# RedhawkSDR/psk_soft

Measured on AMD Instinct MI355X. Metric: complex IQ Msamples/s, QPSK 8 sps, 4096 ch; % HBM roofline at 1/2/4/8 GPUs, higher is better.
Workload: dtype f32

## Files before the change

### psk_soft_amd/csrc/psk_capi.cpp

```cpp
#include <hip/hip_runtime_api.h>
#include <hip/hip_vector_types.h>

#include <atomic>
#include <cmath>
#include <condition_variable>
#include <cstdio>
#include <cstdlib>
#include <cstring>
#include <functional>
#include <mutex>
#include <new>
#include <string>
#include <thread>
#include <vector>

#include "psk_acquire.h"
#include "psk_ctl.h"
#include "psk_gather.h"
#include "psk_plan.h"
#include "psk_quality.h"
#include "psk_soft_hip.h"
#include "psk_tune.h"

namespace psk {
// ... 369 lines not shown
    hipStream_t up_stream = nullptr;
    hipEvent_t ev_up[kPlanSlots] = {};
    int opt_up_stream = 1;
    bool ev_used[kPlanSlots] = {};
    int slot = 0;
    bool opt_qpsk_sign_map = false;
    hipStream_t stream = nullptr;
    hipStream_t aux[kAuxStreams] = {};
    hipEvent_t aux_fork = nullptr, aux_join[kAuxStreams] = {};
    int opt_fork = 1;
    int opt_deferred = 0;
    bool deferred_pending = false;
    uint64_t deferred_sig = 0;
    uint32_t deferred_ch0 = 0, deferred_nch = 0;
    hipStream_t deferred_stream = nullptr;
    hipEvent_t slot_aux_ev[kPlanSlots][kAuxStreams] = {};
    bool slot_aux_used[kPlanSlots][kAuxStreams] = {};
    hipStream_t slot_stream[kPlanSlots] = {};
    uint32_t slot_ch0[kPlanSlots] = {}, slot_nch[kPlanSlots] = {};
    int opt_tiled = 1;
    psk::TileInfo *d_tiles = nullptr;
    float *d_traw = nullptr, *d_test = nullptr;
    float2 *d_ts = nullptr;
    size_t tile_cap = 0, tile_sym_cap = 0;
    size_t pf_cap = 0, pf_sym_cap = 0;
    psk::PfScratch pf{};
    int opt_pfit = 1;
    int pf_second_ttl = 0;
    int opt_ties_in_place = 1;
    int opt_trace = 0;
    int opt_validate = 0;
    int opt_split = 2;
    int opt_pipe = 1;
    hipStream_t pipe_st[2] = {};
    hipEvent_t pipe_ev[kPipeEvents] = {};
    void *d_pipe_carry = nullptr;
    float *d_pipe_y = nullptr;
    size_t pipe_cap = 0;
    void *d_wide_rec = nullptr, *d_wide_stat = nullptr;
    size_t wide_rec_cap = 0, wide_stat_cap = 0;
    double *d_wide_symE = nullptr;
    size_t wide_symE_cap = 0;
    hipEvent_t tile_ev = nullptr;
    hipStream_t tile_stream = nullptr;
    bool tile_ev_used = false;
    int opt_far_fit = 0;
    float *d_far_y = nullptr;
    uint32_t far_rows_cap = 0, far_rows_used = 0;
    std::vector<uint32_t> far_row;
    bool poisoned = false;
    StreamScratch cvt[kCvtScratch];
    uint64_t cvt_calls = 0;
    StreamScratch gat[kGatherScratch];
    GatherDescSlot gdesc[kGatherDescSlots];
    uint64_t gat_calls = 0;
    int gdesc_turn = 0;
    float *d_tune_tab = nullptr;
    int opt_diag_gather_only = 0;
    int opt_quality = 0;
    psk_soft_quality_t *d_quality = nullptr;
    std::vector<psk_soft_quality_t> quality_dry;
    PassRing<psk::QualityDesc, psk::QualityPartial, kQualitySlots> qpass;
    struct QualitySnap {
        uint16_t M, S;
        uint8_t diff;
    };
// ... 988 lines not shown
    float *const carry_y = h->d_pipe_y + (size_t)kPipeMaxYLen * s.off;
    const uint32_t y_pipe = ring_floats(s.max_n, 512u);
    int e = 0;
    PSK_HIP(hipEventRecord(h->pipe_ev[e], st));
    PSK_HIP(hipStreamWaitEvent(h->pipe_st[0], h->pipe_ev[e], 0));
    PSK_HIP(hipStreamWaitEvent(h->pipe_st[1], h->pipe_ev[e], 0));
    e++;
    for (uint32_t t0 = 0; t0 < T; t0 += tr) {
        const uint32_t nt = T - t0 < tr ? T - t0 : tr;
        PSK_HIP(mark(r, st, "pipe_front", S, H, s.off, cnt, nt, y_len, r_len));
        PSK_HIP(psk::launch_tile_front(S, class_H(H), r.d_plans, l, r.ch0, cnt, nt, h->d_state, h->d_ring, h->lim.ring_cap, r_len, h->d_tiles,
                                       h->d_traw, h->d_ts, h->pf.chan, t0, st));
        PSK_HIP(hipEventRecord(h->pipe_ev[e], st));
        PSK_HIP(hipStreamWaitEvent(h->pipe_st[0], h->pipe_ev[e], 0));
        e++;
        PSK_HIP(mark(r, h->pipe_st[0], "pipe_fit", S, H, s.off, cnt, nt, y_pipe, 0));
        PSK_HIP(psk::launch_tile_fit_range(r.d_plans, l, r.ch0, cnt, h->d_state, h->d_ring, h->lim.ring_cap, h->d_yv, h->lim.fit_cap, y_pipe,
                                           h->d_tiles, h->d_traw, h->d_ts, h->d_test, carry, carry_y, t0, nt, h->pipe_st[0]));
        PSK_HIP(hipEventRecord(h->pipe_ev[e], h->pipe_st[0]));
        PSK_HIP(hipStreamWaitEvent(h->pipe_st[1], h->pipe_ev[e], 0));
        e++;
        PSK_HIP(mark(r, h->pipe_st[1], "pipe_back", S, H, s.off, cnt, nt, y_pipe, 0));
        PSK_HIP(psk::launch_tile_back(r.d_plans, l, r.ch0, cnt, nt, h->d_state, h->d_tiles, h->d_ts, h->d_test, t0, 1u, h->pipe_st[1]));
    }
    PSK_HIP(hipEventRecord(h->pipe_ev[e], h->pipe_st[1]));
    PSK_HIP(hipStreamWaitEvent(st, h->pipe_ev[e], 0));
    return PSK_SOFT_OK;
}
psk_soft_status enqueue_class(const Round &r, int S, int H, hipStream_t st)
{
    psk_soft_handle *const h = r.h;
    const LaunchSet &s = r.res.cls[S][H];
    const uint32_t *const l = r.d_list + s.off;
    const uint32_t y_len = ring_floats(s.max_n, psk::ering_dynamic(S) ? 256u : 512u);
    const uint32_t r_len = class_H(H) == 1 ? ((s.max_A + 128u + 1u) & ~1u) : 0u;
    if (s.tiled && s.piped)
        PSK_TRY(enqueue_piped(r, s, S, H, y_len, r_len, st));
    else if (s.tiled)
        PSK_TRY(enqueue_tiled(r, s, {"tile_front", "pfit", "tile_fit", "tile_back", S, H, y_len, r_len, r_len}, Front::window_class, Fit::lds, st));
    const psk::PktFormat *const f = class_pkt(H);
    for (int exact = s.tiled ? 1 : 0; exact <= 1; exact++) {
        if (exact && diag_no_tail())
            break;
        PSK_HIP(mark(r, st, exact ? "fast (exact tier)" : "fast (screened tier)", S, H, s.off, s.cnt, 0, y_len, r_len));
        if (f)
            PSK_HIP(psk::launch_fast_pkt((int)f->id, S, exact, r.d_plans, l, r.ch0, s.cnt, h->d_state, h->d_ring, h->lim.ring_cap, h->d_yv,
                                         h->lim.fit_cap, y_len, r_len, st));
        else
            PSK_HIP(psk::launch_fast(S, class_H(H), exact, r.d_plans, l, r.ch0, s.cnt, h->d_state, h->d_ring, h->lim.ring_cap, h->d_yv,
                                     h->lim.fit_cap, y_len, r_len, st));
    }
    if (r.deferred && f)
        PSK_HIP(psk::launch_seq_pkt((int)f->id, r.d_plans, l, r.ch0, s.cnt, h->d_state, h->d_ring, h->lim.ring_cap, h->d_yv, h->lim.fit_cap, st));
    else if (r.deferred)
        PSK_HIP(psk::launch_seq(r.d_plans, l, r.ch0, s.cnt, h->d_state, h->d_ring, h->lim.ring_cap, h->d_yv, h->lim.fit_cap, st));
    return PSK_SOFT_OK;
}
psk_soft_status enqueue_join_and_tail(Round &r, int used_aux)
{
    psk_soft_handle *const h = r.h;
    const hipStream_t st = r.stream;
    if (r.deferred) {
        for (int a = 0; a < used_aux && a < kAuxStreams; a++) {
            if (!h->slot_aux_ev[r.slot][a])
                PSK_HIP(hipEventCreateWithFlags(&h->slot_aux_ev[r.slot][a], hipEventDisableTiming));
            PSK_HIP(hipEventRecord(h->slot_aux_ev[r.slot][a], h->aux[a]));
            h->slot_aux_used[r.slot][a] = true;
// ... 183 lines not shown
    h->nch = n_channels;
    h->user = lim;
    h->lim.ring_cap = lim.max_window_samples;
    h->lim.fit_cap = lim.max_phase_avg + 1;
    h->lim.fast_fit_max = kFastFitMax;
    h->lim.force_seq = false;
    h->lim.far_fit = false;
    h->ctl.resize(n_channels);
    h->ctl_next.resize(n_channels);
    h->last_mode.assign(n_channels, psk::PLAN_SKIP);
    h->device = device;
    h->dry = (device == PSK_SOFT_DEVICE_NONE);
    if (h->dry) {
        h->quality_dry.assign(n_channels, psk_soft_quality_t{});
        h->acquire_dry.assign(n_channels, psk_soft_acquire_t{});
    }
    if (const char *e = std::getenv("PSK_SOFT_TIME_TILED"))
        h->opt_tiled = std::atoi(e) < 0 ? 0 : std::atoi(e) > 2 ? 2 : std::atoi(e);
    if (const char *e = std::getenv("PSK_SOFT_FAR_FIT"))
        h->opt_far_fit = std::atoi(e) != 0;
    h->lim.far_fit = h->opt_far_fit != 0;
    if (const char *e = std::getenv("PSK_SOFT_TIES_IN_PLACE"))
        h->opt_ties_in_place = std::atoi(e) != 0;
    if (const char *e = std::getenv("PSK_SOFT_TRACE_LAUNCHES"))
        h->opt_trace = std::atoi(e);
    if (const char *e = std::getenv("PSK_SOFT_VALIDATE"))
        h->opt_validate = std::atoi(e);
    if (const char *e = std::getenv("PSK_SOFT_DIAG_GATHER_ONLY"))
        h->opt_diag_gather_only = std::atoi(e) != 0;
    if (const char *e = std::getenv("PSK_SOFT_SPLIT_CLASSES"))
        h->opt_split = std::atoi(e) < 0 ? 0 : std::atoi(e) > 16 ? 16 : std::atoi(e);
    if (const char *e = std::getenv("PSK_SOFT_PIPELINED"))
        h->opt_pipe = std::atoi(e) < 0 ? 0 : std::atoi(e) > 2 ? 2 : std::atoi(e);
    if (const char *e = std::getenv("PSK_SOFT_DEFERRED_JOIN"))
        h->opt_deferred = std::atoi(e) != 0;
    if (const char *e = std::getenv("PSK_SOFT_STAMP"))
        h->opt_stamp = std::atoi(e) != 0;
    if (const char *e = std::getenv("PSK_SOFT_PARALLEL_FIT"))
        h->opt_pfit = std::atoi(e) < 0 ? 0 : std::atoi(e) > 2 ? 2 : std::atoi(e);
    if (!h->dry) {
        int ndev = 0;
        hipError_t e = hipGetDeviceCount(&ndev);
        if (e != hipSuccess || ndev <= 0 || device < 0 || device >= ndev) {
            delete h;
            return fail(PSK_SOFT_ERR_NO_DEVICE,
                        std::string("psk_soft_create: no usable HIP device (") +
                            (e != hipSuccess ? hipGetErrorString(e) : "device index out of range") + ")");
        }
        hipDeviceProp_t prop;
        if (hipSetDevice(device) != hipSuccess || hipGetDeviceProperties(&prop, device) != hipSuccess) {
            delete h;
            return fail(PSK_SOFT_ERR_NO_DEVICE, "psk_soft_create: hipSetDevice failed");
        }
        if (std::strncmp(prop.gcnArchName, "gfx950", 6) != 0) {
            delete h;
            return fail(PSK_SOFT_ERR_NO_DEVICE,
                        std::string("psk_soft_create: kernels are built for gfx950 only, device is ") + prop.gcnArchName);
        }
        auto bail = [&](const char *what, hipError_t e2) {
            std::string msg = std::string("psk_soft_create: ") + what + ": " + hipGetErrorString(e2);
            psk_soft_destroy(h);
            return fail(PSK_SOFT_ERR_HIP, msg);
        };
        hipError_t e2;
        if ((e2 = hipStreamCreateWithFlags(&h->stream, hipStreamNonBlocking)) != hipSuccess)
            return bail("hipStreamCreate", e2);
        size_t state_b = sizeof(psk::ChanState) * (size_t)n_channels;
        size_t ring_b = sizeof(float2) * 2u * (size_t)h->lim.ring_cap * n_channels;
        size_t yv_b = sizeof(float) * (size_t)h->lim.fit_cap * n_channels;
        if ((e2 = hipMalloc((void **)&h->d_state, state_b)) != hipSuccess) return bail("hipMalloc state", e2);
        if ((e2 = hipMalloc((void **)&h->d_ring, ring_b)) != hipSuccess) return bail("hipMalloc ring", e2);
        if ((e2 = hipMalloc((void **)&h->d_yv, yv_b)) != hipSuccess) return bail("hipMalloc yvals", e2);
        std::vector<psk::ChanState> init(n_channels);
        std::memset(init.data(), 0, state_b);
        for (auto &s : init) s.lf_den = 1.0f;
        if ((e2 = hipMemcpy(h->d_state, init.data(), state_b, hipMemcpyHostToDevice)) != hipSuccess)
            return bail("hipMemcpy state", e2);
        if ((e2 = hipMemset(h->d_ring, 0, ring_b)) != hipSuccess) return bail("hipMemset", e2);
        if ((e2 = hipMemset(h->d_yv, 0, yv_b)) != hipSuccess) return bail("hipMemset", e2);
        if ((e2 = hipMalloc((void **)&h->d_quality, sizeof(psk_soft_quality_t) * (size_t)n_channels)) != hipSuccess)
            return bail("hipMalloc quality", e2);
        if ((e2 = hipMemset(h->d_quality, 0, sizeof(psk_soft_quality_t) * (size_t)n_channels)) != hipSuccess) return bail("hipMemset", e2);
        if ((e2 = hipMalloc((void **)&h->d_acquire, sizeof(psk_soft_acquire_t) * (size_t)n_channels)) != hipSuccess)
            return bail("hipMalloc acquire", e2);
        if ((e2 = hipMemset(h->d_acquire, 0, sizeof(psk_soft_acquire_t) * (size_t)n_channels)) != hipSuccess) return bail("hipMemset", e2);
        for (int s = 0; s < kPlanSlots; s++) {
            char *hb = nullptr, *db = nullptr;
            if ((e2 = hipHostMalloc((void **)&hb, slot_bytes(n_channels))) != hipSuccess)
                return bail("hipHostMalloc plans", e2);
            std::memset(hb, 0, psk::kPlanHeaderBytes);
            h->h_plans[s] = reinterpret_cast<psk::ChanPlan *>(hb + psk::kPlanHeaderBytes);
// ... 1450 lines not shown
```

### psk_soft_amd/csrc/psk_fast_kernel.h

```cpp
#ifndef PSK_FAST_KERNEL_H
#define PSK_FAST_KERNEL_H

#include <mutex>

#include "psk_fast_loop.h"

namespace psk {

PSK_HD int hist_blocks_for(uint32_t A) { return A <= 128u ? 1 : A <= 256u ? 2 : A <= 512u ? 4 : 8; }

template <bool FAR = false>
PSK_DEV void call_prologue(const ChanPlan &p, const ChanState *st, const float *yv, uint32_t fit_cap, float *yring, uint32_t ymask,
                           int lane, FastCarry &cy)
{
    const uint32_t len0 = p.lf_len0;
    for (uint32_t j = lane; j < len0; j += kWave) yring[j & ymask] = yv[(p.lf_head + j) % fit_cap];
    if constexpr (FAR)
        far_ring_fence();
    else
        wave_lds_fence();
    cy.ySum = st->lf_ySum;
    cy.xySum = st->lf_xySum;
    cy.est = st->phaseEstimate;
    cy.last_re = st->last_re;
// ... 85 lines not shown
            st->stat_chain = cy.stat_chain;
            st->stat_pfit = 0u;
        }
    }
}

#ifndef PSK_WAVES_PER_SIMD
#define PSK_WAVES_PER_SIMD 4
#endif
#ifndef PSK_WAVES_PER_SIMD_H0
#define PSK_WAVES_PER_SIMD_H0 2
#endif
#ifndef PSK_WAVES_PER_SIMD_H2
#define PSK_WAVES_PER_SIMD_H2 1
#endif
template <int SV, int HV, bool EXACT>
__global__ __launch_bounds__(64, ((HV == 0 && SV <= 5 && !EXACT) ? 4 : (HV == 0 && SV <= 10 && !EXACT) ? PSK_WAVES_PER_SIMD_H0 : (HV == 1 && SV <= 10 && !EXACT) ? PSK_WAVES_PER_SIMD : (HV == 2 && SV <= 10 && !EXACT) ? PSK_WAVES_PER_SIMD_H2 : (HV == 4 && SV <= 8 && !EXACT && PSK_DBUF) ? 2 : 1)) void psk_fast_kernel(const ChanPlan *__restrict__ plans, const uint32_t *__restrict__ list, uint32_t ch0,
                                                      ChanState *__restrict__ states, float2 *__restrict__ rings,
                                                      uint32_t ring_cap, float *__restrict__ yvs, uint32_t fit_cap,
                                                      uint32_t y_len, uint32_t r_len)
{
    extern __shared__ __attribute__((aligned(16))) float lds_dyn[];
    constexpr bool kDyn = ering_dynamic(SV);
    float *const yring = lds_dyn;
    const uint32_t ymask = y_len - 1u;
    ERingT<kDyn> er;
    if constexpr (kDyn) {
        er.mem = lds_dyn + y_len;
        er.set_len((int)r_len);
    } else {
        __shared__ __attribute__((aligned(16))) float ering_s[(SV != 0 && HV == 1) ? SV * kERing : 4];
        er.mem = ering_s;
    }
    const int lane = threadIdx.x & 63;
#ifdef PSK_DIAG_STAMP
    const uint32_t diag_t0 = (uint32_t)wall_clock64();
#endif
#ifdef PSK_STAGGER
    if (SV != 0 && !EXACT) {
        const uint32_t hsh = (blockIdx.x * 2654435761u) >> 24;
        for (uint32_t i = 0; i < (hsh * (uint32_t)(PSK_STAGGER)) >> 8; i++) __builtin_amdgcn_s_sleep(16);
    }
#endif
    if constexpr (EXACT) {
        if (plan_header(plans)[0] == 0u)
            return;
    }
    const uint32_t bi = list[blockIdx.x];
    const ChanPlan &p = plans[bi];
    if (p.mode != PLAN_FAST)
        return;
    if (SV == 0 ? (p.n_out != 0) : (p.n_out == 0 || p.S != (uint32_t)SV || (HV == 0 ? p.A <= (uint32_t)kB : hist_blocks_for(p.A) != HV)))
        return;
    if (EXACT && states[ch0 + bi].guard != 1u)
        return;
    if (!EXACT && SV != 0 && (p.lf_flags & PLAN_TILED) && states[ch0 + bi].guard != 1u)
        return;
    const uint32_t ch = ch0 + bi;
    ChanState *st = &states[ch];
    float2 *ring_base = rings + (size_t)ch * 2u * ring_cap;
    const float2 *ring_src = ring_base + (size_t)p.ring_src * ring_cap;
    float2 *ring_dst = ring_base + (size_t)(p.ring_src ^ 1u) * ring_cap;
    float *yv = yvs + (size_t)ch * fit_cap;

    XView X;
    X.ring = reinterpret_cast<const f2g *>(ring_src);
    X.in = reinterpret_cast<const pkt_t *>(p.in);
    X.L0 = p.ring_len0;

    FastCarry cy;
    call_prologue(p, st, yv, fit_cap, yring, ymask, lane, cy);
#ifdef PSK_DIAG_STAMP2
    const uint32_t diag_t1 = (uint32_t)wall_clock64();
#endif

    if constexpr (SV != 0) {
        const float carried = (p.lf_flags & PLAN_CARRY_DRIFT) ? __uint_as_float(st->pad_state) : 0.0f;
        fast_main_loop<SV, HV, EXACT>(p, X, yring, ymask, er, cy, 0, -1, nullptr, nullptr, carried >= 0.0f ? carried : __builtin_inff());
        if (lane == 0)
            st->pad_state = __float_as_uint(cy.wmax * 1.00001f);
        if constexpr (PSK_PACE_ON(false, EXACT))
            pace_post(pace_key(), 0u, lane);
    }

#ifdef PSK_DIAG_STAMP2
    const uint32_t diag_t2 = (uint32_t)wall_clock64();
#endif
    {
        unsigned umax = wave_max_u32(cy.umax);
        unsigned umin1 = wave_min_u32(cy.umin1);
        if (umin1 != 0xFFFFFFFFu && __any(cy.ambiguous)) {
            int emax = (int)(umax >> 23), emin = (int)((umin1 + 1u) >> 23);
            emax = emax < 1 ? 1 : emax;
            emin = emin < 1 ? 1 : emin;
            int terms_log2 = 32 - __builtin_clz((unsigned)(p.A + 2u * kB));
            if (24 + (emax - emin) + terms_log2 > 52)
                cy.refuse = true;
        }
        cy.refuse = __any(cy.refuse);
    }
    if (cy.refuse) {
        if (lane == 0) {
            st->guard = 1u;
            if (!EXACT)
#ifdef PSK_HANDOVER_VIA_ARG
                atomicAdd(plan_header(plans), 1u);
#else
                atomicAdd(p.handed_over, 1u);
#endif
        }
        return;
// ... 62 lines not shown
```

### psk_soft_amd/csrc/psk_fast_loop.h

```cpp
#ifndef PSK_FAST_LOOP_H
#define PSK_FAST_LOOP_H

#include "psk_wave.h"

namespace psk {

constexpr int kR = 2;
constexpr int kB = kWave * kR;
constexpr int kMaxUnwrapPasses = 160;
#ifndef PSK_TIES_IN_PLACE
#define PSK_TIES_IN_PLACE 1
#endif
#ifndef PSK_WIDE_FIRST
#define PSK_WIDE_FIRST 1
#endif
#ifndef PSK_DBUF
#define PSK_DBUF 1
#endif
constexpr int kScreenRefresh = 64;

struct FastCarry {
    double ySum, xySum;
    float est;
    float last_re, last_im;
// ... 185 lines not shown
        for (int k = 0; k < S; k++) {
            const u2g t = q[k];
            const f2g a = pkt_f2(t.x), b = pkt_f2(t.y);
            x[(2 * k) / S][(2 * k) % S] = make_float2(a.x, a.y);
            x[(2 * k + 1) / S][(2 * k + 1) % S] = make_float2(b.x, b.y);
        }
        return;
#else
        const f2g *base = X.in + ((uint64_t)tau_first * (uint64_t)S - (uint64_t)X.L0);
        const typename F4Ptr<packet_global(S)>::type q =
            (typename F4Ptr<packet_global(S)>::type)base + (uint32_t)lane * (uint32_t)S;
#pragma unroll
        for (int k = 0; k < S; k++) {
#if PSK_NT_LOAD
            const f4g t = __builtin_nontemporal_load(q + k);
#else
            const f4g t = q[k];
#endif
            x[(2 * k) / S][(2 * k) % S] = make_float2(t.x, t.y);
            x[(2 * k + 1) / S][(2 * k + 1) % S] = make_float2(t.z, t.w);
        }
        return;
#endif
    }
#pragma unroll
    for (int r = 0; r < kR; r++) {
        const long long tau = cblk * kB + 2 * lane + r + (long long)A - 1;
        const bool ok = tau >= tau_lo && tau <= tau_hi;
        load_symbol_any<S>(X, (uint64_t)(ok ? tau : 0), ok, x[r]);
    }
}

constexpr int kERing = 2 * kB;
template <bool DYN>
struct ERingT;
template <>
struct ERingT<false> {
    float *mem;
    PSK_DEV void set_len(int) {}
    PSK_DEV int length() const { return kERing; }
    PSK_DEV int wrap(int i) const { return i & (kERing - 1); }
    PSK_DEV float *row(int k) const { return mem + k * kERing; }
};
template <>
struct ERingT<true> {
    float *mem;
    int len;
    PSK_DEV void set_len(int r) { len = r; }
    PSK_DEV int length() const { return len; }
    PSK_DEV int wrap(int i) const { return i < 0 ? i + len : (i >= len ? i - len : i); }
    PSK_DEV float *row(int k) const { return mem + k * len; }
};
template <int S>
PSK_DEV void ering_put(const ERingT<ering_dynamic(S)> &er, int base, int lane, const float (&e)[kR][S])
{
    const int i = er.wrap(base + 2 * lane);
#pragma unroll
    for (int k = 0; k < S; k++) *reinterpret_cast<float2 *>(er.row(k) + i) = make_float2(e[0][k], e[1][k]);
}
template <int S>
PSK_DEV void ering_get(const ERingT<ering_dynamic(S)> &er, int base, int lane, uint32_t D, float (&e)[kR][S])
{
    const int i0 = er.wrap(base + 2 * lane - (int)D);
    if ((D & 1u) == 0) {
#pragma unroll
        for (int k = 0; k < S; k++) {
// ... 550 lines not shown
        guard_track<false>(cy, en.x);
        guard_track<false>(cy, en.y);
        guard_track<false>(cy, ep.x);
        guard_track<false>(cy, ep.y);
        guard_track<false>(cy, eo0);
        guard_track<false>(cy, eo1);
        const double Wc = wave_sum_f64((in0 ? (double)ep.x : 0.0) + (in1 ? (double)ep.y : 0.0));
        const double d0 = (double)en.x - (double)eo0, d1 = (double)en.y - (double)eo1;
        const double W1 = Wc + wave_scan_f64(d0 + d1);
        const double W0 = W1 - d1;
        if (first) {
            argtop_first(top[0], W0);
            argtop_first(top[1], W1);
            top[0].k = top[1].k = k;
            first = false;
        } else {
            argtop_next(top[0], W0, k);
            argtop_next(top[1], W1, k);
        }
    }
#pragma unroll
    for (int r = 0; r < kR; r++) {
        if (fail[r]) {
            bestK[r] = top[r].k;
            cy.ambiguous = cy.ambiguous || argtop_ambiguous(top[r], bound_abs);
            if constexpr (FRONT) {
                const float g = top[r].gap / bound_rel;
                cy.gap_rel = (g < cy.gap_rel) ? g : ((g == g) ? cy.gap_rel : 0.0f);
            }
        }
    }
}

template <bool EXACT, bool FAR = false>
PSK_DEV void fit_stage(int c, int lane, uint32_t n, float xd, float den_s, float xavg_s, const FitKnown &fk, const bool (&valid)[kR],
                       const float (&raw)[kR], int nvalid, int lane_last, int r_last, float *yring, uint32_t ymask, FastCarry &cy,
                       float (&est)[kR], const float *z_far = nullptr)
{
    const uint32_t q0 = cy.q;
    float y[kR];
    double ySum_l[kR], xySum_l[kR];
    float den_last = den_s, xavg_last = xavg_s;
    int pass, rejected = 0;
    float m_lane = 0.0f;
    const bool warm = !__builtin_expect(q0 >= n && n != 1u, 1);
    const bool cheap = cy.chain_run != 0;
    if (!warm) {
        pass = fit_block<false, EXACT, FAR>(lane, q0, n, xd, den_s, xavg_s, fk, valid, raw, cy, yring, ymask, y, est, ySum_l, xySum_l,
                                lane_last, r_last, den_last, xavg_last, cheap, rejected, m_lane, z_far);
    } else {
        pass = fit_block<true, EXACT, FAR>(lane, q0, n, xd, den_s, xavg_s, fk, valid, raw, cy, yring, ymask, y, est, ySum_l, xySum_l,
                               lane_last, r_last, den_last, xavg_last, cheap, rejected, m_lane, z_far);
    }
#ifdef PSK_ABL_NOCHAIN
    rejected = 0;
#endif
    if (rejected) {
        if (!warm)
            fit_sums_chain<false, FAR>((rejected & 1) != 0, lane, lane_last, q0, n, xd, fk.sizef, cy.ySum, cy.xySum, valid, yring, ymask, y, ySum_l, xySum_l, z_far);
        else
            fit_sums_chain<true, FAR>(true, lane, lane_last, q0, n, xd, fk.sizef, cy.ySum, cy.xySum, valid, yring, ymask, y, ySum_l, xySum_l, z_far);
        float est2[kR];
#pragma unroll
        for (int r = 0; r < kR; r++) {
            float m_, b_;
            if (!warm) {
                est2[r] = fit_value_known(ySum_l[r], xySum_l[r], fk, m_);
            } else {
                const uint32_t before = q0 + (uint32_t)(2 * lane + r);
                const uint32_t pts = before < n ? before + 1 : n;
                float den_r = den_s, xavg_r = xavg_s;
                if (pts > 1 && pts < n)
                    fit_denominator(xd, pts, den_r, xavg_r);
                est2[r] = pts > 1 ? fit_value(ySum_l[r], xySum_l[r], xd, pts, den_r, xavg_r, m_, b_) : y[r];
            }
        }
        const float fb0 = wave_up1(est2[1], cy.est), old_fb0 = wave_up1(est[1], cy.est);
        const bool diff0 = valid[0] && __float_as_uint(fb0) != __float_as_uint(old_fb0);
        const bool diff1 = valid[1] && __float_as_uint(est2[0]) != __float_as_uint(est[0]);
        if (__any(diff0 || diff1)) {
            const bool moved0 = diff0 && unwrap_count(fb0, (double)raw[0], c) != unwrap_count(old_fb0, (double)raw[0], c);
            const bool moved1 = diff1 && unwrap_count(est2[0], (double)raw[1], c) != unwrap_count(est[0], (double)raw[1], c);
// ... 142 lines not shown
#ifndef PSK_PACE_EVERY
#define PSK_PACE_EVERY 4
#endif
constexpr int kPaceRows = 2048, kPaceSlots = 8;
static __device__ uint32_t g_pace_table[kPaceRows * kPaceSlots];
PSK_DEV uint32_t pace_key()
{
    const uint32_t hw = (uint32_t)__builtin_amdgcn_s_getreg((31 << 11) | 4);
    const uint32_t xcc = (uint32_t)__builtin_amdgcn_s_getreg((3 << 11) | 20);
    const uint32_t r = ((xcc & 7u) << 8) | (((hw >> 13) & 3u) << 6) | (((hw >> 8) & 15u) << 2) | ((hw >> 4) & 3u);
    return (r * (uint32_t)kPaceSlots) | ((hw & 7u) << 16);
}
PSK_DEV uint32_t pace_fetch(uint32_t key, int lane)
{
    uint32_t v = 0u;
    if (lane < kPaceSlots)
        v = __hip_atomic_load(g_pace_table + (key & 0xffffu) + lane, __ATOMIC_RELAXED, __HIP_MEMORY_SCOPE_AGENT);
    return v;
}
PSK_DEV void pace_post(uint32_t key, uint32_t left, int lane)
{
    if (lane == 0)
        __hip_atomic_store(g_pace_table + (key & 0xffffu) + (key >> 16), left, __ATOMIC_RELAXED, __HIP_MEMORY_SCOPE_AGENT);
}
PSK_DEV int pace_rank(uint32_t key, uint32_t row_word, uint32_t left, int lane)
{
    const unsigned long long more = __builtin_amdgcn_ballot_w64(lane < kPaceSlots && lane != (int)(key >> 16) && row_word > left);
    const int ahead = __builtin_popcountll(more);
    return ahead >= 3 ? 0 : 3 - ahead;
}

template <int S, int H, bool EXACT, bool FRONT = false>
PSK_DEV void fast_main_loop(const ChanPlan &p, const XView &X, float *yring, uint32_t ymask, const ERingT<ering_dynamic(S)> &er, FastCarry &cy,
                            int c_begin = 0, int c_end = -1, float *t_raw = nullptr, float2 *t_s = nullptr, float wmax_floor = 0.0f)
{

    const int lane = threadIdx.x & 63;
    const uint32_t A = p.A, M = p.M, n = p.lf_n;
    const int n_out = (int)p.n_out;
#define g_soft mem_ptr<packet_global(S)>(p.soft)
#define g_phase mem_ptr<packet_global(S)>(p.phase)
#define g_bits mem_ptr<packet_global(S)>(p.bits)
#define g_sidx mem_ptr<packet_global(S)>(p.sidx)
    const float xd = p.lf_xdelta;
    const long long tau_last = (long long)n_out + (long long)A - 2;

    constexpr bool REREAD = (H == 0);
    BlockKeep<S> hist[H ? H : 1];
    double Wc[S];
    float Wf[S];
    if constexpr (REREAD) {
        static_assert(!REREAD || !EXACT, "the exact tier keeps its history in registers");
        double acc[S];
#pragma unroll
        for (int k = 0; k < S; k++) acc[k] = 0.0;
        for (int h = (int)((A + 126u) / (uint32_t)kB) - 1; h >= 0; h--) {
            float2 x[kR][S];
            load_block<S>(X, (long long)c_begin - (long long)(h + 1), A, (long long)c_begin * kB, (long long)c_begin * kB + (long long)A - 2, lane, x);
#pragma unroll
            for (int r = 0; r < kR; r++) {
#pragma unroll
                for (int k = 0; k < S; k++) acc[k] += (double)norm_f(x[r][k].x, x[r][k].y);
            }
        }
#pragma unroll
        for (int k = 0; k < S; k++) {
            Wc[k] = wave_sum_f64(acc[k]);
            Wf[k] = uni((float)Wc[k]);
        }
    } else {
        double acc[S];
#pragma unroll
        for (int k = 0; k < S; k++) acc[k] = 0.0;
#pragma unroll
        for (int h = H - 1; h >= 0; h--) {
            float2 x[kR][S];
            load_block<S>(X, (long long)c_begin - (long long)(h + 1), A, (long long)c_begin * kB, (long long)c_begin * kB + (long long)A - 2, lane, x);
#pragma unroll
            for (int r = 0; r < kR; r++) {
#pragma unroll
                for (int k = 0; k < S; k++) {
                    float e = norm_f(x[r][k].x, x[r][k].y);
                    if (EXACT)
                        guard_track<true>(cy, e);
                    hist[h].e[r][k] = e;
                    acc[k] += (double)e;
                }
                hist[h].kp[r] = (int)cy.last_k;
                hist[h].pk[r] = select_sample<S>(x[r], (int)cy.last_k);
            }
        }
#pragma unroll
        for (int k = 0; k < S; k++) {
            Wc[k] = wave_sum_f64(acc[k]);
            Wf[k] = uni((float)Wc[k]);
        }
    }
    const float kU = 5.9604645e-08f;
    float wmax_prev = 0.0f;
#pragma unroll
    for (int k = 0; k < S; k++) wmax_prev = __builtin_fmaxf(wmax_prev, Wf[k]);
    wmax_prev = __builtin_fmaxf(wmax_prev, wmax_floor);
    if constexpr (EXACT)
        cy.wmax = __builtin_fmaxf(cy.wmax, wmax_floor);
    float err_c = 2.0f * kU * wmax_prev;
    const float c_blk = uni(kU * (64.0f + 16.0f * ((float)kB / (float)A + 1.0f)));
    int since_refresh = 0;

    const RotParam rotE = rot_param(lane, A);
    const RotParam rotP = rot_param(lane, A - 1);
    const int uE = (H <= 1) ? 0 : rotE.u, uP = (H <= 1) ? 0 : rotP.u;

    float den_s = cy.den, xavg_s = cy.xavg;
    if (n > 1)
        fit_denominator(xd, n, den_s, xavg_s);
    const FitKnown fk = fit_known(xd, n, den_s, xavg_s);
    const bool m_pow2 = M != 0 && (M & (M - 1)) == 0;
    const float inv_M = uni(1.0f / (float)(M ? M : 1));

    const int n_blocks = (FRONT && c_end >= 0) ? c_end : (n_out + kB - 1) / kB;
    const AtanTabDev atab = atan_tab_dev(lane);
    const bool qpsk_sign_map = (p.lf_flags & PLAN_QPSK_SIGN_MAP) != 0;
    int kpred[kR] = {(int)cy.last_k, (int)cy.last_k};

    int ring_base = 0;
    if constexpr (H == 1)
        ering_put<S>(er, er.length() - kB, lane, hist[0].e);

    constexpr uint32_t kPaceBias = (PSK_WIDE_FIRST && H >= 2) ? (1u << 24) : 0u;
    uint32_t pace = 0u;
    if constexpr (PSK_PACE_ON(FRONT, EXACT))
        pace = pace_key();
    auto set_prio_dyn = [](int v) {
        switch (v) {
        case 0: __builtin_amdgcn_s_setprio(0); break;
        case 1: __builtin_amdgcn_s_setprio(1); break;
        case 2: __builtin_amdgcn_s_setprio(2); break;
        default: __builtin_amdgcn_s_setprio(3); break;
        }
    };
    constexpr bool DBUF = PSK_DBUF && H >= 2 && !FRONT && !EXACT;
    float2 xnext[kR][S];
    if constexpr (DBUF) {
        if (c_begin < n_blocks)
            load_block<S>(X, (long long)c_begin, A, 0, tau_last, lane, xnext);
    }
#if PSK_PACE_SHORT_MODE == 2
    const int pace_mask = n_blocks <= PSK_PACE_SHORT ? 0 : PSK_PACE_EVERY - 1;
#endif
    for (int c = c_begin; c < n_blocks; c++) {
        if constexpr (!PSK_PACE_ON(FRONT, EXACT))
// ... 105 lines not shown
        }
        if constexpr (!REREAD) {
            float nx[kR], ox[kR], ny[kR], oy[kR];
            int nk[kR], ok2[kR];
#pragma unroll
            for (int rr = 0; rr < kR; rr++) {
                nx[rr] = block_back<S, H>(uP, cur, hist, [&](const BlockKeep<S> &b) { return b.pk[rr].x; });
                ox[rr] = block_back<S, H>(uP + 1, cur, hist, [&](const BlockKeep<S> &b) { return b.pk[rr].x; });
                ny[rr] = block_back<S, H>(uP, cur, hist, [&](const BlockKeep<S> &b) { return b.pk[rr].y; });
                oy[rr] = block_back<S, H>(uP + 1, cur, hist, [&](const BlockKeep<S> &b) { return b.pk[rr].y; });
                nk[rr] = block_back<S, H>(uP, cur, hist, [&](const BlockKeep<S> &b) { return b.kp[rr]; });
                ok2[rr] = block_back<S, H>(uP + 1, cur, hist, [&](const BlockKeep<S> &b) { return b.kp[rr]; });
            }
#pragma unroll
            for (int r = 0; r < kR; r++) {
                px[r] = rot_pull<float>(rotP, r, nx, ox);
                py[r] = rot_pull<float>(rotP, r, ny, oy);
                pkk[r] = rot_pull<int>(rotP, r, nk, ok2);
            }
        }

        int bestK[kR] = {0, 0};
        if constexpr (!EXACT) {
            constexpr int IB = S <= 2 ? 1 : S <= 4 ? 2 : S <= 8 ? 3 : S <= 16 ? 4 : 5;
            constexpr int IMASK = (1 << IB) - 1;
            float inc[S], d1v[S];
#pragma unroll
            for (int k = 0; k < S; k++) {
                const float d0 = cur.e[0][k] - e_old[0][k];
                d1v[k] = cur.e[1][k] - e_old[1][k];
                inc[k] = d0 + d1v[k];
            }
            wave_scan_f32_multi(inc);
            int m1[kR], m2[kR];
            int nz = 0;
#pragma unroll
            for (int k = 0; k < S; k++) {
                const float W1 = Wf[k] + inc[k];
                const float W0 = W1 - d1v[k];
                nz |= __float_as_int(W0) | __float_as_int(W1);
                Wf[k] = read_lane(W1, 63);
                const int p0 = (__float_as_int(W0) & (0x7FFFFFFF & ~IMASK)) | (IMASK - k);
                const int p1 = (__float_as_int(W1) & (0x7FFFFFFF & ~IMASK)) | (IMASK - k);
                if (k == 0) {
                    m1[0] = p0;
                    m1[1] = p1;
                } else if (k == 1) {
                    m2[0] = p0 < m1[0] ? p0 : m1[0];
                    m2[1] = p1 < m1[1] ? p1 : m1[1];
                    m1[0] = p0 > m1[0] ? p0 : m1[0];
                    m1[1] = p1 > m1[1] ? p1 : m1[1];
                } else {
                    m2[0] = med3_i32(m1[0], m2[0], p0);
                    m2[1] = med3_i32(m1[1], m2[1], p1);
                    m1[0] = p0 > m1[0] ? p0 : m1[0];
                    m1[1] = p1 > m1[1] ? p1 : m1[1];
                }
            }
            bestK[0] = IMASK - (m1[0] & IMASK);
            bestK[1] = IMASK - (m1[1] & IMASK);
            const int mm = m1[0] > m1[1] ? m1[0] : m1[1];
            const float wmax = __builtin_fmaxf(wave_max_f32(__int_as_float(mm)), wmax_prev);
            const float e_blk = c_blk * wmax;
            const float thr_floor = vote_any((nz & 0x7FFFFFFF) != 0) ? (float)(16 << IB) * 1.4012985e-45f : 0.0f;
            const float thr = 6.0f * (err_c + e_blk) + (float)(4 << IB) * kU * wmax + thr_floor;
            const bool ok0 = !valid[0] || ((__int_as_float(m1[0]) - __int_as_float(m2[0])) > thr);
            const bool ok1 = !valid[1] || ((__int_as_float(m1[1]) - __int_as_float(m2[1])) > thr);
            if constexpr (FRONT) {
                if (__any((valid[0] && ok0) || (valid[1] && ok1))) {
                    const float cap_blk = thr / (2.0f * drift_bound(c * kB + kB, A));
                    cy.cap = cap_blk < cy.cap ? cap_blk : cy.cap;
                }
            }
            err_c += e_blk;
            wmax_prev = wmax;
            since_refresh++;
            if (!__all(ok0 && ok1)) {
                if constexpr (H == 1) {
                    const bool fail[kR] = {!ok0, !ok1};
                    const float best_f[kR] = {__int_as_float(m1[0]), __int_as_float(m1[1])};
                    const int second_k[kR] = {IMASK - (m2[0] & IMASK), IMASK - (m2[1] & IMASK)};
                    const int sym0 = (p.lf_flags & PLAN_CARRY_DRIFT) ? (int)p.count0 : 0;
                    exact_block_from_ring<S, FRONT>(er, ring_base, A, lane, cy, bestK,
                                                    2.0f * drift_bound(sym0 + c * kB + kB, A) * wmax_prev, fail, best_f, second_k, thr,
                                                    2.0f * drift_bound(sym0 + c * kB + kB, A));
                    since_refresh = kScreenRefresh;
                    cy.stat_exact_blocks += 1;
                } else if (PSK_TIES_IN_PLACE && !(p.lf_flags & PLAN_TIES_HANDOVER)) {
                    double Wst[S];
                    if constexpr (REREAD)
                        window_end_reread_f64<S>(X, c - 1, c_begin, A, tau_last, lane, cy, Wst);
                    else
                        window_end_f64<S, H>(hist, A, lane, cy, Wst);
                    ArgTop top[kR];
#pragma unroll
                    for (int k = 0; k < S; k++) {
// ... 91 lines not shown
            }
        }

        if constexpr (!REREAD) {
#pragma unroll
            for (int h = H - 1; h > 0; h--) hist[h] = hist[h - 1];
            hist[0] = cur;
        }

        if constexpr (PSK_PACE_ON(FRONT, EXACT)) {
        } else if (cy.chain_streak >> 16)
            __builtin_amdgcn_s_setprio(PSK_CHAIN_PRIO);
        else
            __builtin_amdgcn_s_setprio(0);
        float raw[kR];
#pragma unroll
        for (int r = 0; r < kR; r++) {
            cf32 pw = cpow_uint<EXACT>(s[r], M);
            if (!EXACT && valid[r] && !(is_fin(pw.re) && is_fin(pw.im)))
                cy.refuse = true;
            raw[r] = atan2f_wave(pw.im, pw.re, atab);
        }

        if constexpr (FRONT) {
            *reinterpret_cast<float2 *>(t_raw + i0) = make_float2(raw[0], raw[1]);
            *reinterpret_cast<float4 *>(t_s + i0) = make_float4(s[0].re, s[0].im, s[1].re, s[1].im);
            cy.stat_blocks += 1;
            if (__any(cy.refuse)) {
                cy.refuse = true;
                return;
            }
        } else {
        float est[kR];
        fit_stage<EXACT>(c, lane, n, xd, den_s, xavg_s, fk, valid, raw, nvalid, lane_last, r_last, yring, ymask, cy, est);
        if constexpr (!EXACT) {
            if (__any(cy.refuse)) {
                cy.refuse = true;
                return;
            }
        }

        {
            cf32 last_c;
            last_c.re = cy.last_re;
            last_c.im = cy.last_im;
            output_stage<packet_global(S), EXACT>(p, c, i0, valid, s, est, last_c, atab, qpsk_sign_map, m_pow2, inv_M);
        }
        if (p.diff) {
            const float sre = r_last ? s[1].re : s[0].re;
            const float sim = r_last ? s[1].im : s[0].im;
            cy.last_re = read_lane(sre, lane_last);
            cy.last_im = read_lane(sim, lane_last);
        }
        }

        if constexpr (!EXACT) {
            if (since_refresh >= kScreenRefresh) {
                float wm = 0.0f;
                float wre[S];
                if constexpr (REREAD)
                    window_end_reread_f32<S>(X, c, c_begin, A, tau_last, lane, wre);
#pragma unroll
                for (int k = 0; k < S; k++) {
                    if constexpr (REREAD)
                        Wf[k] = wre[k];
                    else if constexpr (H == 1)
                        Wf[k] = window_end_ring_f32(er, ring_base, A, lane, k);
                    else
                        Wf[k] = window_end_f32<S, H>(hist, A, lane, k);
                    wm = __builtin_fmaxf(wm, Wf[k]);
                }
                wmax_prev = __builtin_fmaxf(wmax_prev, wm);
                err_c = (REREAD ? (float)(8u + 2u * ((A + 127u) / (uint32_t)kB)) : 16.0f) * kU * wmax_prev;
                since_refresh = 0;
            }
        }
        if constexpr (H == 1)
            ring_base = er.wrap(ring_base + kB);
    }
    if constexpr (!EXACT)
        cy.wmax = wmax_prev;
}

#undef g_soft
#undef g_phase
#undef g_bits
#undef g_sidx
}
#endif
```

Before: 478,300.

## Park loop-invariant fit state in LDS and shrink y-ring for large H=1 classes

In the screened fast kernel for static-ring H=1 classes, the running window values Wf, the FitKnown constants, c_blk and inv_M are kept in shared memory instead of registers. The aim is to lower VGPR pressure and raise occupancy. Separately, untiled H=1 classes whose channel count exceeds 15 per CU now use a 256-entry y-ring instead of 512, cutting ring memory traffic and footprint. The cost is extra LDS reads and writes inside the hot loop, plus possible extra ring wraps.

```diff
diff --git a/psk_soft_amd/csrc/psk_capi.cpp b/psk_soft_amd/csrc/psk_capi.cpp
--- a/psk_soft_amd/csrc/psk_capi.cpp
+++ b/psk_soft_amd/csrc/psk_capi.cpp
@@ -425,6 +425,8 @@
     int opt_validate = 0;
     int opt_split = 2;
     int opt_pipe = 1;
+    int opt_small_ring = 1;
+    uint32_t small_ring_above = 15u * 256u;
     hipStream_t pipe_st[2] = {};
     hipEvent_t pipe_ev[kPipeEvents] = {};
     void *d_pipe_carry = nullptr;
@@ -1479,7 +1481,9 @@
     psk_soft_handle *const h = r.h;
     const LaunchSet &s = r.res.cls[S][H];
     const uint32_t *const l = r.d_list + s.off;
-    const uint32_t y_len = ring_floats(s.max_n, psk::ering_dynamic(S) ? 256u : 512u);
+    const bool small_ring = psk::ering_dynamic(S) || (class_H(H) == 1 && !s.tiled && h->opt_small_ring &&
+                                                      (h->opt_small_ring == 2 || s.cnt > h->small_ring_above));
+    const uint32_t y_len = ring_floats(s.max_n, small_ring ? 256u : 512u);
     const uint32_t r_len = class_H(H) == 1 ? ((s.max_A + 128u + 1u) & ~1u) : 0u;
     if (s.tiled && s.piped)
         PSK_TRY(enqueue_piped(r, s, S, H, y_len, r_len, st));
@@ -1729,6 +1733,8 @@
         h->opt_split = std::atoi(e) < 0 ? 0 : std::atoi(e) > 16 ? 16 : std::atoi(e);
     if (const char *e = std::getenv("PSK_SOFT_PIPELINED"))
         h->opt_pipe = std::atoi(e) < 0 ? 0 : std::atoi(e) > 2 ? 2 : std::atoi(e);
+    if (const char *e = std::getenv("PSK_SOFT_SMALL_RING"))
+        h->opt_small_ring = std::atoi(e) < 0 ? 0 : std::atoi(e) > 2 ? 2 : std::atoi(e);
     if (const char *e = std::getenv("PSK_SOFT_DEFERRED_JOIN"))
         h->opt_deferred = std::atoi(e) != 0;
     if (const char *e = std::getenv("PSK_SOFT_STAMP"))
@@ -1754,6 +1760,8 @@
             return fail(PSK_SOFT_ERR_NO_DEVICE,
                         std::string("psk_soft_create: kernels are built for gfx950 only, device is ") + prop.gcnArchName);
         }
+        if (prop.multiProcessorCount > 0)
+            h->small_ring_above = 15u * (uint32_t)prop.multiProcessorCount;
         auto bail = [&](const char *what, hipError_t e2) {
             std::string msg = std::string("psk_soft_create: ") + what + ": " + hipGetErrorString(e2);
             psk_soft_destroy(h);
diff --git a/psk_soft_amd/csrc/psk_fast_kernel.h b/psk_soft_amd/csrc/psk_fast_kernel.h
--- a/psk_soft_amd/csrc/psk_fast_kernel.h
+++ b/psk_soft_amd/csrc/psk_fast_kernel.h
@@ -141,6 +141,11 @@
         __shared__ __attribute__((aligned(16))) float ering_s[(SV != 0 && HV == 1) ? SV * kERing : 4];
         er.mem = ering_s;
     }
+    float *park = nullptr;
+    if constexpr (park_on(SV, HV, EXACT)) {
+        __shared__ __attribute__((aligned(16))) float park_s[park_floats(SV)];
+        park = park_s;
+    }
     const int lane = threadIdx.x & 63;
 #ifdef PSK_DIAG_STAMP
     const uint32_t diag_t0 = (uint32_t)wall_clock64();
@@ -185,7 +190,7 @@
 
     if constexpr (SV != 0) {
         const float carried = (p.lf_flags & PLAN_CARRY_DRIFT) ? __uint_as_float(st->pad_state) : 0.0f;
-        fast_main_loop<SV, HV, EXACT>(p, X, yring, ymask, er, cy, 0, -1, nullptr, nullptr, carried >= 0.0f ? carried : __builtin_inff());
+        fast_main_loop<SV, HV, EXACT>(p, X, yring, ymask, er, cy, 0, -1, nullptr, nullptr, carried >= 0.0f ? carried : __builtin_inff(), park);
         if (lane == 0)
             st->pad_state = __float_as_uint(cy.wmax * 1.00001f);
         if constexpr (PSK_PACE_ON(false, EXACT))
diff --git a/psk_soft_amd/csrc/psk_fast_loop.h b/psk_soft_amd/csrc/psk_fast_loop.h
--- a/psk_soft_amd/csrc/psk_fast_loop.h
+++ b/psk_soft_amd/csrc/psk_fast_loop.h
@@ -241,6 +241,10 @@
 }
 
 constexpr int kERing = 2 * kB;
+constexpr bool park_on(int S, int H, bool exact) { return S != 0 && H == 1 && !exact && !ering_dynamic(S); }
+constexpr int park_fit(int S) { return (S + 3) & ~3; }
+constexpr int park_misc(int S) { return park_fit(S) + (int)((sizeof(FitKnown) + 15) / 16) * 4; }
+constexpr int park_floats(int S) { return park_misc(S) + 4; }
 template <bool DYN>
 struct ERingT;
 template <>
@@ -857,7 +861,7 @@
     }
 }
 
-template <bool EXACT, bool FAR = false>
+template <bool EXACT, bool FAR = false, bool PARKED = false>
 PSK_DEV void fit_stage(int c, int lane, uint32_t n, float xd, float den_s, float xavg_s, const FitKnown &fk, const bool (&valid)[kR],
                        const float (&raw)[kR], int nvalid, int lane_last, int r_last, float *yring, uint32_t ymask, FastCarry &cy,
                        float (&est)[kR], const float *z_far = nullptr)
@@ -871,8 +875,8 @@
     const bool warm = !__builtin_expect(q0 >= n && n != 1u, 1);
     const bool cheap = cy.chain_run != 0;
     if (!warm) {
-        pass = fit_block<false, EXACT, FAR>(lane, q0, n, xd, den_s, xavg_s, fk, valid, raw, cy, yring, ymask, y, est, ySum_l, xySum_l,
-                                lane_last, r_last, den_last, xavg_last, cheap, rejected, m_lane, z_far);
+        pass = fit_block<false, EXACT, FAR>(lane, q0, n, PARKED ? fk.xd : xd, den_s, xavg_s, fk, valid, raw, cy, yring, ymask, y, est, ySum_l,
+                                xySum_l, lane_last, r_last, den_last, xavg_last, cheap, rejected, m_lane, z_far);
     } else {
         pass = fit_block<true, EXACT, FAR>(lane, q0, n, xd, den_s, xavg_s, fk, valid, raw, cy, yring, ymask, y, est, ySum_l, xySum_l,
                                lane_last, r_last, den_last, xavg_last, cheap, rejected, m_lane, z_far);
@@ -1081,7 +1085,8 @@
 
 template <int S, int H, bool EXACT, bool FRONT = false>
 PSK_DEV void fast_main_loop(const ChanPlan &p, const XView &X, float *yring, uint32_t ymask, const ERingT<ering_dynamic(S)> &er, FastCarry &cy,
-                            int c_begin = 0, int c_end = -1, float *t_raw = nullptr, float2 *t_s = nullptr, float wmax_floor = 0.0f)
+                            int c_begin = 0, int c_end = -1, float *t_raw = nullptr, float2 *t_s = nullptr, float wmax_floor = 0.0f,
+                            float *park = nullptr)
 {
 
     const int lane = threadIdx.x & 63;
@@ -1095,6 +1100,7 @@
     const long long tau_last = (long long)n_out + (long long)A - 2;
 
     constexpr bool REREAD = (H == 0);
+    constexpr bool PARK = park_on(S, H, EXACT) && !FRONT;
     BlockKeep<S> hist[H ? H : 1];
     double Wc[S];
     float Wf[S];
@@ -1149,6 +1155,10 @@
     float wmax_prev = 0.0f;
 #pragma unroll
     for (int k = 0; k < S; k++) wmax_prev = __builtin_fmaxf(wmax_prev, Wf[k]);
+    if constexpr (PARK) {
+#pragma unroll
+        for (int k = 0; k < S; k++) park[k] = Wf[k];
+    }
     wmax_prev = __builtin_fmaxf(wmax_prev, wmax_floor);
     if constexpr (EXACT)
         cy.wmax = __builtin_fmaxf(cy.wmax, wmax_floor);
@@ -1164,8 +1174,14 @@
     if (n > 1)
         fit_denominator(xd, n, den_s, xavg_s);
     const FitKnown fk = fit_known(xd, n, den_s, xavg_s);
+    if constexpr (PARK)
+        *reinterpret_cast<FitKnown *>(park + park_fit(S)) = fk;
     const bool m_pow2 = M != 0 && (M & (M - 1)) == 0;
     const float inv_M = uni(1.0f / (float)(M ? M : 1));
+    if constexpr (PARK) {
+        park[park_misc(S)] = c_blk;
+        park[park_misc(S) + 1] = inv_M;
+    }
 
     const int n_blocks = (FRONT && c_end >= 0) ? c_end : (n_out + kB - 1) / kB;
     const AtanTabDev atab = atan_tab_dev(lane);
@@ -1337,14 +1353,20 @@
                 inc[k] = d0 + d1v[k];
             }
             wave_scan_f32_multi(inc);
+            float wf[S];
+#pragma unroll
+            for (int k = 0; k < S; k++) wf[k] = PARK ? park[k] : Wf[k];
             int m1[kR], m2[kR];
             int nz = 0;
 #pragma unroll
             for (int k = 0; k < S; k++) {
-                const float W1 = Wf[k] + inc[k];
+                const float W1 = wf[k] + inc[k];
                 const float W0 = W1 - d1v[k];
                 nz |= __float_as_int(W0) | __float_as_int(W1);
-                Wf[k] = read_lane(W1, 63);
+                if constexpr (PARK)
+                    wf[k] = W1;
+                else
+                    Wf[k] = read_lane(W1, 63);
                 const int p0 = (__float_as_int(W0) & (0x7FFFFFFF & ~IMASK)) | (IMASK - k);
                 const int p1 = (__float_as_int(W1) & (0x7FFFFFFF & ~IMASK)) | (IMASK - k);
                 if (k == 0) {
@@ -1362,11 +1384,17 @@
                     m1[1] = p1 > m1[1] ? p1 : m1[1];
                 }
             }
+            if constexpr (PARK) {
+                if (lane == kWave - 1) {
+#pragma unroll
+                    for (int k = 0; k < S; k++) park[k] = wf[k];
+                }
+            }
             bestK[0] = IMASK - (m1[0] & IMASK);
             bestK[1] = IMASK - (m1[1] & IMASK);
             const int mm = m1[0] > m1[1] ? m1[0] : m1[1];
             const float wmax = __builtin_fmaxf(wave_max_f32(__int_as_float(mm)), wmax_prev);
-            const float e_blk = c_blk * wmax;
+            const float e_blk = (PARK ? park[park_misc(S)] : c_blk) * wmax;
             const float thr_floor = vote_any((nz & 0x7FFFFFFF) != 0) ? (float)(16 << IB) * 1.4012985e-45f : 0.0f;
             const float thr = 6.0f * (err_c + e_blk) + (float)(4 << IB) * kU * wmax + thr_floor;
             const bool ok0 = !valid[0] || ((__int_as_float(m1[0]) - __int_as_float(m2[0])) > thr);
@@ -1524,7 +1552,11 @@
             }
         } else {
         float est[kR];
-        fit_stage<EXACT>(c, lane, n, xd, den_s, xavg_s, fk, valid, raw, nvalid, lane_last, r_last, yring, ymask, cy, est);
+        if constexpr (PARK)
+            fit_stage<EXACT, false, true>(c, lane, n, xd, den_s, xavg_s, *reinterpret_cast<const FitKnown *>(park + park_fit(S)), valid, raw, nvalid,
+                                          lane_last, r_last, yring, ymask, cy, est);
+        else
+            fit_stage<EXACT>(c, lane, n, xd, den_s, xavg_s, fk, valid, raw, nvalid, lane_last, r_last, yring, ymask, cy, est);
         if constexpr (!EXACT) {
             if (__any(cy.refuse)) {
                 cy.refuse = true;
@@ -1536,7 +1568,7 @@
             cf32 last_c;
             last_c.re = cy.last_re;
             last_c.im = cy.last_im;
-            output_stage<packet_global(S), EXACT>(p, c, i0, valid, s, est, last_c, atab, qpsk_sign_map, m_pow2, inv_M);
+            output_stage<packet_global(S), EXACT>(p, c, i0, valid, s, est, last_c, atab, qpsk_sign_map, m_pow2, PARK ? park[park_misc(S) + 1] : inv_M);
         }
         if (p.diff) {
             const float sre = r_last ? s[1].re : s[0].re;
@@ -1561,6 +1593,8 @@
                     else
                         Wf[k] = window_end_f32<S, H>(hist, A, lane, k);
                     wm = __builtin_fmaxf(wm, Wf[k]);
+                    if constexpr (PARK)
+                        park[k] = Wf[k];
                 }
                 wmax_prev = __builtin_fmaxf(wmax_prev, wm);
                 err_c = (REREAD ? (float)(8u + 2u * ((A + 127u) / (uint32_t)kB)) : 16.0f) * kU * wmax_prev;
```

Result: slower. 455,100 (-4.9%).
